# ForeverFancy/GVFDiffusion

Hardware: AMD Instinct MI355X
Metric: 4D frames/sec (800x800x24f, 256k Gaussians) + DiT denoise steps/sec (higher is better)
Workload: dtype f32

## Files before the change

gvfdiffusion_amd/csrc/rast.hip:

```cpp
#include <atomic>
#include <cstdlib>
#include <mutex>
#include <type_traits>
#include <vector>
#include "gvf_common.h"
#include "gvf_sort.h"
#include "../../include/gvf_rast.h"

namespace {

constexpr int PRE_THREADS = 256;
constexpr int NSLAB = 1;
#ifndef GVF_PRE_FB
#define GVF_PRE_FB 4
#endif
constexpr int PRE_FB = GVF_PRE_FB;
#ifndef GVF_PRE_XCD
#define GVF_PRE_XCD 0
#endif
#ifndef GVF_PRE_REC_QUAD
#define GVF_PRE_REC_QUAD 1
#endif
#ifndef GVF_PRE_PREFETCH
#define GVF_PRE_PREFETCH 0
// ... 31 lines not shown
    const float s1 = __builtin_fmaf(-l11, px, __builtin_fmaf(-l12, py, c1));
    const float s2 = __builtin_fmaf(-l22, py, c2);
    return __builtin_fmaf(s2, s2, __builtin_fmaf(s1, s1, -lo));
}

__constant__ float SH_C0 = 0.28209479177387814f;
__constant__ float SH_C1 = 0.4886025119029199f;
__constant__ float SH_C2[5] = {1.0925484305920792f, -1.0925484305920792f, 0.31539156525252005f,
                               -1.0925484305920792f, 0.5462742152960396f};
__constant__ float SH_C3[7] = {-0.5900435899266435f, 2.890611442640554f, -0.4570457994644658f,
                               0.3731763325901154f, -0.4570457994644658f, 1.445305721320277f,
                               -0.5900435899266435f};

struct PreParams {
    int P, M, deg, H, W, mode;
    int gx, gy;
    float kernel_size, scale_modifier;
    int fused;
    GvfGaussianActivation act;
    int n_delta;
    int upstream_binning;
    int F;
    int delta_lds;
};

__device__ __forceinline__ float act_expf(float x) {
    if (x != x) return x;
    if (x > 88.72283f) return __builtin_inff();
    if (x < -103.97208f) return 0.0f;
    const float kf = x * 1.44269502f + (x < 0.0f ? -0.5f : 0.5f);
    const int k = (int)kf;
    const float t = (float)k;
    float r = __builtin_fmaf(t, -0.693145751953125f, x);
    r = __builtin_fmaf(t, -1.42860677e-6f, r);
    float p = 1.98412698e-4f;
    p = __builtin_fmaf(p, r, 1.38888889e-3f);
    p = __builtin_fmaf(p, r, 8.33333377e-3f);
    p = __builtin_fmaf(p, r, 4.16666679e-2f);
    p = __builtin_fmaf(p, r, 1.66666672e-1f);
    p = __builtin_fmaf(p, r, 0.5f);
    p = __builtin_fmaf(p, r, 1.0f);
    p = __builtin_fmaf(p, r, 1.0f);
    const int k1 = k / 2, k2 = k - k1;
    return (p * __uint_as_float((uint32_t)(k1 + 127) << 23)) * __uint_as_float((uint32_t)(k2 + 127) << 23);
}
__device__ __forceinline__ float act_log1pf(float y) {
// ... 226 lines not shown
__device__ __forceinline__ void tight_range(float c, float h, int lo, int hi, int n, int& t0, int& t1) {
    if (h < 0.0f) { t0 = lo; t1 = lo; return; }
    const float a = fminf(fmaxf(ceilf((c - h - (float)(TILE - 1)) / (float)TILE), 0.0f), (float)n);
    const float b = fminf(fmaxf(floorf((c + h) / (float)TILE) + 1.0f, 0.0f), (float)n);
    t0 = max((int)a, lo);
    t1 = min((int)b, hi);
    if (t1 < t0) t1 = t0;
}

__device__ __forceinline__ TileRect tight_rect(TileRect r, float px, float py, float hx, float hy, int gx, int gy) {
    TileRect t;
    tight_range(px, hx, r.x0, r.x1, gx, t.x0, t.x1);
    tight_range(py, hy, r.y0, r.y1, gy, t.y0, t.y1);
    return t;
}

template <bool SHARED>
__global__ __launch_bounds__(PRE_THREADS) void preprocess_kernel(
    PreParams pp, const GvfRastFrame* __restrict__ frames, const float* __restrict__ a0,
    const float* __restrict__ a1, const float* __restrict__ a2, const float* __restrict__ a3,
    const float* __restrict__ sh, const float* __restrict__ colors_precomp,
    const float* __restrict__ cov3D_precomp, const float* __restrict__ delta, float4* __restrict__ splats,
    uint32_t* __restrict__ tiles_touched,
    int32_t* __restrict__ radii, uint32_t* __restrict__ block_sums, uint4* __restrict__ binrec,
    const uint32_t* __restrict__ bin_slot ,
    const float2* __restrict__ zrange ) {
    extern __shared__ __attribute__((aligned(16))) float sh_lds[];
    const int t = threadIdx.x;
    const int P = pp.P, M = pp.M;
    const int nbx = (P + PRE_THREADS - 1) / PRE_THREADS;
    int bx = blockIdx.x, by = blockIdx.y;
    if (GVF_PRE_XCD) {
        const int FY = (pp.F + PRE_FB - 1) / PRE_FB, k = (int)(blockIdx.x >> 3);
        bx = (k / FY) * 8 + (int)(blockIdx.x & 7u);
        by = k - (k / FY) * FY;
        if (bx >= nbx) return;
    }
    const int i = bx * PRE_THREADS + t;

    const int sh_stride = M * 3;
    if (sh != nullptr) {
        const size_t span0 = (size_t)bx * PRE_THREADS * sh_stride;
        const int nvalid = min(PRE_THREADS, P - bx * PRE_THREADS);
        const int total = nvalid * sh_stride;
        const float4* src4 = reinterpret_cast<const float4*>(sh + span0);
        float4* dst4 = reinterpret_cast<float4*>(sh_lds);
        const int n4 = total >> 2;
// ... 224 lines not shown
        const size_t o = (size_t)f * P + i;
#if defined(PRE_ABL_NOREC)
        if (touched != 0 && gA.x == 12345.678f) splats[4 * o] = gA;
#else
        if (!GVF_PRE_REC_QUAD && touched != 0) {
            float4* rec = splats + 4 * o;
            rec[0] = gA; rec[1] = gB; rec[2] = gC;
        }
#endif
        if (tiles_touched != nullptr) tiles_touched[o] = touched;
        if (radii != nullptr) {
            const uint32_t* gid_of = SHARED ? reinterpret_cast<const uint32_t*>(a1) : nullptr;
            radii[gid_of != nullptr ? (size_t)f * P + gid_of[i] : o] = radius_out;
        }
        if (binrec != nullptr) {
            uint32_t slab = 0u;
            if (zrange != nullptr) {
                const float2 zr = zrange[f];
                slab = (uint32_t)fminf(fmaxf((gC.y - zr.x) * zr.y, 0.0f), (float)(NSLAB - 1));
            }
#if defined(PRE_ABL_NOBIN)
            if (gC.y == 12345.678f)
#endif
            binrec[(size_t)f * P + my_slot] = make_uint4((uint32_t)rect.x0 | ((uint32_t)rect.y0 << 16),
                                                         (uint32_t)rect.x1 | ((uint32_t)rect.y1 << 16), __float_as_uint(gC.y), slab);
        }
    }

#if !defined(PRE_ABL_NOREC)
    if (GVF_PRE_REC_QUAD) {
        const int lj = t & 3;
        float4* qbase = splats + 4 * ((size_t)f * P + (size_t)(i & ~3));
#define GVF_QB(v_, k_) __builtin_bit_cast(float, __builtin_amdgcn_mov_dpp(__builtin_bit_cast(int, (v_)), (k_) * 0x55, 0xF, 0xF, true))
#define GVF_QSTORE(k_)                                                                                          \
        {                                                                                                       \
            const int tk = __builtin_amdgcn_mov_dpp((int)touched, (k_) * 0x55, 0xF, 0xF, true);                 \
            float4 o4;                                                                                          \
            { const float a = GVF_QB(gA.x, k_), b = GVF_QB(gB.x, k_), c = GVF_QB(gC.x, k_); o4.x = lj == 0 ? a : (lj == 1 ? b : (lj == 2 ? c : 0.f)); } \
            { const float a = GVF_QB(gA.y, k_), b = GVF_QB(gB.y, k_), c = GVF_QB(gC.y, k_); o4.y = lj == 0 ? a : (lj == 1 ? b : (lj == 2 ? c : 0.f)); } \
            { const float a = GVF_QB(gA.z, k_), b = GVF_QB(gB.z, k_), c = GVF_QB(gC.z, k_); o4.z = lj == 0 ? a : (lj == 1 ? b : (lj == 2 ? c : 0.f)); } \
            { const float a = GVF_QB(gA.w, k_), b = GVF_QB(gB.w, k_), c = GVF_QB(gC.w, k_); o4.w = lj == 0 ? a : (lj == 1 ? b : (lj == 2 ? c : 0.f)); } \
            if (tk != 0) qbase[4 * (k_) + lj] = o4;                                                             \
        }
        GVF_QSTORE(0) GVF_QSTORE(1) GVF_QSTORE(2) GVF_QSTORE(3)
#undef GVF_QSTORE
#undef GVF_QB
    }
#endif
// ... 180 lines not shown
    float lo[3], hi[3];
#pragma unroll
    for (int k = 0; k < 3; ++k) {
        lo[k] = float_unordered(mm[k]); hi[k] = float_unordered(mm[3 + k]);
        if (fused) { lo[k] = lo[k] * act.aabb[3 + k] + act.aabb[k]; hi[k] = hi[k] * act.aabb[3 + k] + act.aabb[k]; }
        if (lo[k] > hi[k]) { const float tmp = lo[k]; lo[k] = hi[k]; hi[k] = tmp; }
    }
    const float* V = frames[f].viewmatrix;
    float zmin = 3.0e38f, zmax = -3.0e38f;
    for (int c = 0; c < 8; ++c) {
        const float p[3] = {(c & 1) ? hi[0] : lo[0], (c & 2) ? hi[1] : lo[1], (c & 4) ? hi[2] : lo[2]};
        const float z = V[2] * p[0] + V[6] * p[1] + V[10] * p[2] + V[14];
        zmin = fminf(zmin, z); zmax = fmaxf(zmax, z);
    }
    zmin = fmaxf(zmin, 0.2f);
    const float ext = fmaxf(zmax - zmin, 1e-6f);
    zrange[f] = make_float2(zmin - 0.02f * ext, (float)NSLAB / (1.04f * ext));
}

constexpr int WIN_MAX = 2048;
constexpr int BIN_SPT = 4;
constexpr int BIN_SLOTS = PRE_THREADS * BIN_SPT;

template <bool SCATTER>
__global__ __launch_bounds__(PRE_THREADS) void bin_kernel(int P, int gx, int gy, const uint4* __restrict__ binrec,
                                                          const uint32_t* __restrict__ order,
                                                          uint32_t* __restrict__ tile_count ,
                                                          uint32_t* __restrict__ cursor ,
                                                          const uint32_t* __restrict__ total,
                                                          uint64_t* __restrict__ payload, int nslab,
                                                          const uint32_t* __restrict__ frame_base, uint32_t* __restrict__ num_rendered,
                                                          int rec_by_id, int xcd_frames, int F) {
    __shared__ uint32_t s_tab[WIN_MAX];
    __shared__ uint32_t s_run[SCATTER ? WIN_MAX : 1];
    __shared__ int s_box[4];
    int blk = (int)blockIdx.x, f = (int)blockIdx.y;
    if (xcd_frames) {
        const int nblk = (P + BIN_SLOTS - 1) / BIN_SLOTS, k = (int)(blockIdx.x >> 3);
        f = (k / nblk) * 8 + (int)(blockIdx.x & 7u);
        blk = k - (k / nblk) * nblk;
        if (f >= F) return;
    }
    if (SCATTER && num_rendered != nullptr && blk == 0 && threadIdx.x == 0)
        num_rendered[f] = frame_base[f + 1] - frame_base[f];
    if (SCATTER && *total == 0u) return;
    const int t = threadIdx.x, lane = t & 63;
    if (t == 0) { s_box[0] = 0x7fffffff; s_box[1] = 0x7fffffff; s_box[2] = 0; s_box[3] = 0; }
    int x0[BIN_SPT], y0[BIN_SPT], x1[BIN_SPT], y1[BIN_SPT], sl[BIN_SPT];
    uint64_t key[BIN_SPT];
    int bx0 = 0x7fffffff, by0 = 0x7fffffff, bx1 = 0, by1 = 0;
#pragma unroll
    for (int k = 0; k < BIN_SPT; ++k) {
        const int s = blk * BIN_SLOTS + k * PRE_THREADS + t;
        x0[k] = y0[k] = x1[k] = y1[k] = 0; sl[k] = 0; key[k] = 0;
        if (s < P) {
            const uint32_t id = order != nullptr ? order[s] : (uint32_t)s;
            const uint4 br = binrec[(size_t)f * P + (rec_by_id ? id : (uint32_t)s)];
            x0[k] = (int)(br.x & 0xffffu); y0[k] = (int)(br.x >> 16);
            x1[k] = (int)(br.y & 0xffffu); y1[k] = (int)(br.y >> 16);
            sl[k] = (int)br.w;
            key[k] = ((uint64_t)br.z << 32) | id;
            if (x1[k] > x0[k] && y1[k] > y0[k]) {
                bx0 = min(bx0, x0[k]); by0 = min(by0, y0[k]); bx1 = max(bx1, x1[k]); by1 = max(by1, y1[k]);
            } else {
                x1[k] = x0[k];
            }
        }
    }
#pragma unroll
    for (int d = 32; d >= 1; d >>= 1) {
        bx0 = min(bx0, __shfl_xor(bx0, d, 64)); by0 = min(by0, __shfl_xor(by0, d, 64));
        bx1 = max(bx1, __shfl_xor(bx1, d, 64)); by1 = max(by1, __shfl_xor(by1, d, 64));
    }
    __syncthreads();
    if (lane == 0 && bx1 > bx0) {
        atomicMin(&s_box[0], bx0); atomicMin(&s_box[1], by0); atomicMax(&s_box[2], bx1); atomicMax(&s_box[3], by1);
    }
    __syncthreads();
    const int wx0 = s_box[0], wy0 = s_box[1], ww = s_box[2] - s_box[0], wh = s_box[3] - s_box[1];
    if (ww <= 0 || wh <= 0) return;
// ... 23 lines not shown
                for (int y = y0[k]; y < y1[k]; ++y)
                    for (int x = x0[k]; x < x1[k]; ++x) {
                        const int e = ((y - wy0) * ww + (x - wx0)) * nslab + sl[k];
                        payload[s_tab[e] + atomicAdd(&s_run[e], 1u)] = key[k];
                    }
        }
    } else {
#pragma unroll
        for (int k = 0; k < BIN_SPT; ++k)
            for (int y = y0[k]; y < y1[k]; ++y)
                for (int x = x0[k]; x < x1[k]; ++x) {
                    const uint32_t pos = atomicAdd(&gtab[(y * gx + x) * nslab + sl[k]], 1u);
                    if (SCATTER) payload[pos] = key[k];
                }
    }
}

constexpr int BINX_THREADS = 512;
constexpr int BINX_TAB = 4096;
constexpr int BINX_PER_WG = 8192;
constexpr int BINX_SPT = 4;

template <bool SCATTER>
__global__ __launch_bounds__(BINX_THREADS) void bin_index_kernel(int P, int gx, const uint4* __restrict__ binrec,
                                                                 uint32_t* __restrict__ tile_count ,
                                                                 uint32_t* __restrict__ cursor ,
                                                                 const uint32_t* __restrict__ total,
                                                                 uint64_t* __restrict__ payload, int nslab, int nseg_frame,
                                                                 const uint32_t* __restrict__ frame_base, uint32_t* __restrict__ num_rendered) {
    __shared__ uint32_t s_tab[BINX_TAB];
    __shared__ uint32_t s_run[SCATTER ? BINX_TAB : 1];
    const int t = threadIdx.x, f = blockIdx.y;
    if (SCATTER && num_rendered != nullptr && blockIdx.x == 0 && t == 0) num_rendered[f] = frame_base[f + 1] - frame_base[f];
    if (SCATTER && *total == 0u) return;
    const int g0 = (int)blockIdx.x * BINX_PER_WG, g1 = min(P, g0 + BINX_PER_WG);
    const uint4* rec = binrec + (size_t)f * P;
    for (int e = t; e < nseg_frame; e += BINX_THREADS) { s_tab[e] = 0u; if (SCATTER) s_run[e] = 0u; }
    __syncthreads();
    auto sweep = [&](auto pass) {
        for (int base = g0; base < g1; base += BINX_SPT * BINX_THREADS) {
            uint4 br[BINX_SPT];
#pragma unroll
            for (int k = 0; k < BINX_SPT; ++k) {
                const int s = base + k * BINX_THREADS + t;
                br[k] = s < g1 ? rec[s] : make_uint4(0u, 0u, 0u, 0u);
            }
#pragma unroll
            for (int k = 0; k < BINX_SPT; ++k) {
                const int x0 = (int)(br[k].x & 0xffffu), y0 = (int)(br[k].x >> 16);
                const int x1 = (int)(br[k].y & 0xffffu), y1 = (int)(br[k].y >> 16);
                const int sl = (int)br[k].w;
                const uint64_t key = ((uint64_t)br[k].z << 32) | (uint32_t)(base + k * BINX_THREADS + t);
                for (int y = y0; y < y1; ++y)
                    for (int x = x0; x < x1; ++x) {
                        const int e = (y * gx + x) * nslab + sl;
                        if constexpr (decltype(pass)::value == 0) atomicAdd(&s_tab[e], 1u);
                        else payload[s_tab[e] + atomicAdd(&s_run[e], 1u)] = key;
                    }
            }
        }
    };
    sweep(std::integral_constant<int, 0>{});
    __syncthreads();
    uint32_t* gtab = (SCATTER ? cursor : tile_count) + (size_t)f * nseg_frame;
    for (int e = t; e < nseg_frame; e += BINX_THREADS) {
        const uint32_t c = s_tab[e];
        if (c != 0u) {
            if (SCATTER) s_tab[e] = atomicAdd(&gtab[e], c);
            else atomicAdd(&gtab[e], c);
        }
    }
    if (SCATTER) {
        __syncthreads();
        sweep(std::integral_constant<int, 1>{});
    }
}

__global__ __launch_bounds__(256) void bbox_kernel(int P, const float* __restrict__ xyz, uint32_t* __restrict__ mm) {
    __shared__ uint32_t s_mm[6];
    if (threadIdx.x < 6) s_mm[threadIdx.x] = threadIdx.x < 3 ? 0xffffffffu : 0u;
    __syncthreads();
    uint32_t lo[3] = {0xffffffffu, 0xffffffffu, 0xffffffffu}, hi[3] = {0u, 0u, 0u};
    for (int i = blockIdx.x * blockDim.x + threadIdx.x; i < P; i += gridDim.x * blockDim.x) {
#pragma unroll
        for (int k = 0; k < 3; ++k) {
            const float v = xyz[3 * (size_t)i + k];
            if (v == v && fabsf(v) < 3.0e38f) {
                const uint32_t o = float_ordered(v);
                lo[k] = min(lo[k], o); hi[k] = max(hi[k], o);
            }
        }
    }
#pragma unroll
    for (int k = 0; k < 3; ++k) {
#pragma unroll
        for (int d = 32; d >= 1; d >>= 1) {
            lo[k] = min(lo[k], (uint32_t)__shfl_xor((int)lo[k], d, 64));
            hi[k] = max(hi[k], (uint32_t)__shfl_xor((int)hi[k], d, 64));
        }
        if ((threadIdx.x & 63) == 0) { atomicMin(&s_mm[k], lo[k]); atomicMax(&s_mm[3 + k], hi[k]); }
    }
    __syncthreads();
    if (threadIdx.x < 3) atomicMin(&mm[threadIdx.x], s_mm[threadIdx.x]);
    else if (threadIdx.x < 6) atomicMax(&mm[threadIdx.x], s_mm[threadIdx.x]);
}

__device__ __forceinline__ uint32_t spread5(uint32_t v) {
    return (v & 1u) | ((v & 2u) << 2) | ((v & 4u) << 4) | ((v & 8u) << 6) | ((v & 16u) << 8);
}

constexpr int MORTON_BINS = 1 << 15;

__device__ __forceinline__ uint32_t morton15(int i, const float* __restrict__ xyz, const uint32_t* __restrict__ mm) {
    uint32_t code = 0;
#pragma unroll
    for (int k = 0; k < 3; ++k) {
        const float lo = float_unordered(mm[k]), hi = float_unordered(mm[3 + k]);
        const float v = xyz[3 * (size_t)i + k];
        float q = (v - lo) / fmaxf(hi - lo, 1e-30f) * 32.0f;
        q = (q == q) ? fminf(fmaxf(q, 0.0f), 31.0f) : 0.0f;
        code |= spread5((uint32_t)q) << k;
    }
    return code;
}

__global__ __launch_bounds__(256) void morton_count_kernel(int P, const float* __restrict__ xyz,
                                                           const uint32_t* __restrict__ mm, uint32_t* __restrict__ codes,
                                                           uint32_t* __restrict__ hist) {
    const int i = blockIdx.x * blockDim.x + threadIdx.x;
    if (i >= P) return;
    const uint32_t c = morton15(i, xyz, mm);
    codes[i] = c;
    atomicAdd(&hist[c], 1u);
}

__global__ __launch_bounds__(1024) void morton_scan_kernel(uint32_t* __restrict__ hist) {
    __shared__ uint32_t wsum[16];
    const int t = threadIdx.x;
    const unsigned lane = t & 63, w = t >> 6;
    constexpr int PER = MORTON_BINS / 1024;
    uint32_t v[PER], s = 0;
#pragma unroll
    for (int k = 0; k < PER; ++k) { v[k] = hist[t * PER + k]; s += v[k]; }
    const uint32_t incl = gvf_wave_incl_scan(s, lane);
    if (lane == 63) wsum[w] = incl;
    __syncthreads();
    uint32_t run = incl - s;
    for (unsigned k = 0; k < w; ++k) run += wsum[k];
#pragma unroll
    for (int k = 0; k < PER; ++k) { hist[t * PER + k] = run; run += v[k]; }
}

__global__ __launch_bounds__(256) void morton_scatter_kernel(int P, uint32_t* codes_rank, uint32_t* __restrict__ hist,
                                                             uint32_t* __restrict__ order) {
    const int i = blockIdx.x * blockDim.x + threadIdx.x;
    if (i >= P) return;
    const uint32_t slot = atomicAdd(&hist[codes_rank[i]], 1u);
    order[slot] = (uint32_t)i;
    codes_rank[i] = slot;
}

__global__ __launch_bounds__(256) void ranges_kernel(const uint64_t* __restrict__ keys,
                                                     const uint32_t* __restrict__ n_ptr, uint32_t n_cap,
                                                     uint2* __restrict__ ranges, uint32_t n_ranges) {
    uint32_t n = *n_ptr;
    n = n < n_cap ? n : n_cap;
    for (uint32_t k = blockIdx.x * blockDim.x + threadIdx.x; k < n; k += gridDim.x * blockDim.x) {
        uint32_t cur = (uint32_t)(keys[k] >> 32);
        if (cur >= n_ranges) continue;
        if (k == 0) ranges[cur].x = 0;
        else {
            uint32_t prev = (uint32_t)(keys[k - 1] >> 32);
            if (cur != prev) { if (prev < n_ranges) ranges[prev].y = k; ranges[cur].x = k; }
        }
        if (k == n - 1) ranges[cur].y = n;
    }
}

#ifndef SORT_BUCKETS
#define SORT_BUCKETS 1
#endif

// ... 680 lines not shown

constexpr int PROF_MAX_CALLS = 256;
constexpr int PROF_EVENTS = GVF_RAST_NSTAGES + 1;
struct Profiler {
    bool on = false;
    std::atomic<int> calls{0};
    hipEvent_t ev[PROF_MAX_CALLS][PROF_EVENTS];
};
Profiler g_prof;
inline void prof_mark(hipStream_t s, int slot, int k) {
    if (slot >= 0) (void)hipEventRecord(g_prof.ev[slot][k], s);
}

struct Workspace {
    GvfRastFrame* frames;
    float4* splats;
    uint32_t* tiles_touched; int32_t* radii;
    uint32_t* block_sums; uint32_t* frame_base; uint32_t* total;
    uint64_t* keys; uint64_t* keys_alt; uint32_t* vals; uint32_t* vals_alt; uint32_t* ids;
    uint2* ranges; uint32_t* cls;
    uint32_t* tile_count; uint32_t* cursor;
    uint32_t* partial; float2* zrange;
    uint32_t* order; uint32_t* order_alt; uint32_t* mhist; uint32_t* mm;
    uint4* binrec;
    void* sort_tmp; size_t sort_tmp_bytes;
    size_t bytes; bool ok;
};

int key_end_bit(int F, int ntiles) {
    uint64_t m = (uint64_t)F * (uint64_t)ntiles;
    int bits = 0;
    while (((uint64_t)1 << bits) < m) ++bits;
    return 32 + bits;
}

Workspace carve(void* ws, size_t bytes, int P, int F, int H, int W, int64_t max_rendered) {
    Workspace w;
    GvfCarver c(ws, bytes);
    const int nb = (P + PRE_THREADS - 1) / PRE_THREADS;
    const int ntiles = ((W + TILE - 1) / TILE) * ((H + TILE - 1) / TILE);
    const size_t FP = (size_t)F * (size_t)(P > 0 ? P : 1);
    const size_t D = (size_t)(max_rendered > 0 ? max_rendered : 1);
    w.frames = c.take<GvfRastFrame>(F);
    w.splats = c.take<float4>(4 * FP);
    w.tiles_touched = c.take<uint32_t>(FP);
    w.radii = c.take<int32_t>(FP);
    w.block_sums = c.take<uint32_t>((size_t)F * (nb > 0 ? nb : 1));
    w.frame_base = c.take<uint32_t>(F + 1);
    w.total = c.take<uint32_t>(1);
    w.keys = c.take<uint64_t>(D);
    w.keys_alt = c.take<uint64_t>(D);
    w.vals = c.take<uint32_t>(D);
    w.vals_alt = c.take<uint32_t>(D);
    w.ids = c.take<uint32_t>(D);
    w.ranges = c.take<uint2>((size_t)F * ntiles * NSLAB);
    w.cls = c.take<uint32_t>(2 + 2 * (size_t)F * ntiles * NSLAB);
    w.tile_count = c.take<uint32_t>((size_t)F * ntiles * NSLAB);
    w.cursor = c.take<uint32_t>((size_t)F * ntiles * NSLAB);
    w.partial = c.take<uint32_t>(((size_t)F * ntiles * NSLAB + SCAN_CHUNK - 1) / SCAN_CHUNK + 1);
    w.zrange = c.take<float2>(F);
    const size_t Pp = (size_t)(P > 0 ? P : 1);
    w.order = c.take<uint32_t>(Pp);
    w.order_alt = c.take<uint32_t>(Pp);
    w.mhist = c.take<uint32_t>(1 << 15);
    w.mm = c.take<uint32_t>(8);
    w.binrec = c.take<uint4>(FP);
    w.sort_tmp_bytes = gvf_sort_tmp_bytes((int64_t)D);
    w.sort_tmp = c.take<char>(w.sort_tmp_bytes);
    w.bytes = gvf_align_up(c.off, 256);
    w.ok = c.ok;
    return w;
}

std::atomic<long long> g_shared_calls{0};

int run_pipeline(const GvfRastSettings& st, const GvfRastFrame* frames_host, int F, int P, int M, bool fused,
                 const GvfGaussianActivation* act, const float* a0, const float* a1, const float* a2,
                 const float* a3, const float* sh, const float* colors_precomp, const float* cov3D_precomp,
                 const float* delta, int n_delta, const float* subpixel_offset, void* workspace,
                 size_t workspace_bytes, int64_t max_rendered, float* out_color, float* out_alpha,
                 float* out_depth, int32_t* out_radii, uint32_t* out_num_rendered, hipStream_t stream,
                 unsigned char* out_u8 = nullptr ) {
    const int H = st.image_height, W = st.image_width;
    if (H <= 0 || W <= 0 || P < 0 || F <= 0 || max_rendered < 0 || max_rendered > 0xFFFFFFFFll) return GVF_EINVAL;
    if (st.sh_degree < 0 || st.sh_degree > 3) return GVF_EINVAL;
    if (st.mode != GVF_RAST_MODE_MIP && st.mode != GVF_RAST_MODE_DILATE) return GVF_EINVAL;
    if ((out_color == nullptr) == (out_u8 == nullptr) || !out_num_rendered || !frames_host || !workspace) return GVF_EINVAL;
    if (P > 0 && colors_precomp == nullptr) {
        if (sh == nullptr || M < (st.sh_degree + 1) * (st.sh_degree + 1) || M > MAX_SH_COEFFS) return GVF_EINVAL;
    }
    (void)hipGetLastError();
    if ((((uintptr_t)sh) & 15) != 0 || (((uintptr_t)workspace) & 255) != 0) return GVF_EINVAL;
    Workspace w = carve(workspace, workspace_bytes, P, F, H, W, max_rendered);
    if (!w.ok) return GVF_ENOSPC;

    const int gx = (W + TILE - 1) / TILE, gy = (H + TILE - 1) / TILE, ntiles = gx * gy;
    const int nb = (P + PRE_THREADS - 1) / PRE_THREADS;
    int slot = g_prof.on ? g_prof.calls.fetch_add(1) : -1;
    if (slot >= PROF_MAX_CALLS) slot = -1;

    ActSlices slices; slices.n = 0;
    bool shared = false;
    std::vector<int> frame_slice((size_t)F, 0);
    const char* shared_env = getenv("GVF_RAST_SHARED_ACT");
    const bool shared_on = !(shared_env && shared_env[0] == '0');
    if (shared_on && fused && cov3D_precomp == nullptr && st.bin_algo != GVF_RAST_BIN_RADIX && P > 0 && F >= 2) {
        shared = true;
        for (int f = 0; f < F && shared; ++f) {
            const int di = (delta != nullptr && frames_host[f].delta_index >= 0) ? frames_host[f].delta_index : -1;
            int k = 0;
            while (k < slices.n && slices.di[k] != di) ++k;
            if (k == slices.n) {
                if (slices.n == ACT_MAX_SLICES) { shared = false; break; }
                slices.di[slices.n++] = di;
            }
            frame_slice[(size_t)f] = k;
        }
        if (shared && (F < 2 * slices.n || (size_t)slices.n * (size_t)P * 64u > (size_t)(max_rendered > 0 ? max_rendered : 0) * 8u)) shared = false;
    }
    const bool index_fits = st.bin_algo != GVF_RAST_BIN_RADIX && !shared && (size_t)ntiles * NSLAB <= (size_t)BINX_TAB;
    const bool index_count = GVF_BIN_ALGO >= 2 && index_fits, index_scatter = GVF_BIN_ALGO == 3 && index_fits;
    const bool morton = st.bin_algo != GVF_RAST_BIN_RADIX && F >= 4 && P >= 4096 && !index_scatter;
    const char* slot_env = getenv("GVF_RAST_SLOT_ORDER");
    const size_t sh_floats = (size_t)(colors_precomp ? 0 : M) * 3;
    const bool slot_mode = shared && !(slot_env && slot_env[0] == '0') && morton && nb > 0 && colors_precomp == nullptr && sh != nullptr &&
                           (size_t)slices.n * (size_t)P * 64u + (size_t)P * sh_floats * 4u <= (size_t)max_rendered * 8u;
    const uint32_t layout = (slot_mode ? LAYOUT_SLOT_ORDER : 0u) | ((uint32_t)((P > 0 && nb > 0 && morton) ? NSLAB : 1) << 8);
    for (int f0 = 0; f0 < F; f0 += 16) {
        FrameChunk ch;
        const int cnt = F - f0 < 16 ? F - f0 : 16;
        for (int k = 0; k < cnt; ++k) {
            ch.f[k] = frames_host[f0 + k];
            ch.f[k].reserved[0] = shared ? frame_slice[(size_t)(f0 + k)] : 0;
        }
        CallTables tab = {};
        if (f0 == 0) {
            const size_t nseg_all = (size_t)F * ntiles * NSLAB;
            tab.ranges = reinterpret_cast<uint32_t*>(w.ranges); tab.n_ranges = (uint32_t)(2 * nseg_all);
            tab.tile_count = w.tile_count; tab.n_tile_count = (uint32_t)nseg_all;
            tab.mhist = w.mhist; tab.n_mhist = morton ? (uint32_t)MORTON_BINS : 0u;
            tab.cls = w.cls; tab.mm = w.mm; tab.layout = layout;
        }
        const size_t clear_words = (size_t)tab.n_ranges + tab.n_tile_count + tab.n_mhist;
        const int zb = f0 == 0 ? (int)((clear_words + 4095) / 4096 < 256 ? (clear_words + 4095) / 4096 : 256) : 0;
        hipLaunchKernelGGL(upload_frames_kernel, dim3(1 + zb), dim3(256), 0, stream, ch, cnt, w.frames + f0, tab);
    }
    GVF_CHECK_LAUNCH();

    int nslab_blend = 1;
    const uint32_t* blend_rec_of = nullptr;
    if (P == 0 || nb == 0) {
        if (hipMemsetAsync(out_num_rendered, 0, sizeof(uint32_t) * F, stream) != hipSuccess) return GVF_ELAUNCH;
    } else {
        const bool bucket = st.bin_algo != GVF_RAST_BIN_RADIX;
        prof_mark(stream, slot, 0);
        const uint32_t* order = nullptr;
        if (morton) {
            int bb = (P + 255) / 256; if (bb > 128) bb = 128;
            const int pb = (P + 255) / 256;
            hipLaunchKernelGGL(bbox_kernel, dim3(bb), dim3(256), 0, stream, P, a0, w.mm);
            hipLaunchKernelGGL(morton_count_kernel, dim3(pb), dim3(256), 0, stream, P, a0, w.mm, w.order_alt, w.mhist);
            hipLaunchKernelGGL(morton_scan_kernel, dim3(1), dim3(1024), 0, stream, w.mhist);
            hipLaunchKernelGGL(morton_scatter_kernel, dim3(pb), dim3(256), 0, stream, P, w.order_alt, w.mhist, w.order);
            order = w.order;
            if (NSLAB > 1)
                hipLaunchKernelGGL(frame_zrange_kernel, dim3((F + 63) / 64), dim3(64), 0, stream, w.frames, F, w.mm, fused ? 1 : 0,
                                   fused ? *act : GvfGaussianActivation{}, w.zrange);
            GVF_CHECK_LAUNCH();
        }
        const int nslab = order != nullptr ? NSLAB : 1;
        const bool rec_gather = GVF_BIN_ALGO >= 1 && bucket && !shared && order != nullptr;
        nslab_blend = nslab;
        const unsigned nseg = (unsigned)((size_t)F * ntiles * nslab);
        prof_mark(stream, slot, 1);
        PreParams pp;
        pp.P = P; pp.M = colors_precomp ? 0 : M; pp.deg = st.sh_degree; pp.H = H; pp.W = W; pp.mode = st.mode;
        pp.gx = gx; pp.gy = gy; pp.kernel_size = st.kernel_size; pp.scale_modifier = st.scale_modifier;
        pp.fused = fused ? 1 : 0; pp.n_delta = n_delta; pp.F = F;
        pp.upstream_binning = (st.upstream_binning != 0 || subpixel_offset != nullptr) ? 1 : 0;
        if (fused) pp.act = *act; else pp.act = GvfGaussianActivation{};
        const size_t sh_lds_bytes = gvf_align_up((size_t)PRE_THREADS * pp.M * 3 * sizeof(float), 16) + 16;
        pp.delta_lds = (GVF_PRE_DELTA_LDS && fused && delta != nullptr && P % 2 == 0 && (((uintptr_t)delta) & 15) == 0) ? 1 : 0;
        const size_t pre_lds_bytes = sh_lds_bytes + (pp.delta_lds ? (size_t)PRE_THREADS * 14 * sizeof(float) : 0);
        const int pre_fy = (F + PRE_FB - 1) / PRE_FB;
        const dim3 pre_grid = GVF_PRE_XCD ? dim3((nb + 7) / 8 * 8 * pre_fy) : dim3(nb, pre_fy);
        if (shared) {
            g_shared_calls.fetch_add(1, std::memory_order_relaxed);
            float4* rec3d = reinterpret_cast<float4*>(w.keys_alt);
            float* sh_by_slot = slot_mode ? reinterpret_cast<float*>(rec3d + 4 * (size_t)slices.n * (size_t)P) : nullptr;
            hipLaunchKernelGGL(activate_cov_kernel, dim3((P + 255) / 256, slices.n), dim3(256), 0, stream, *act, st.scale_modifier, P, slices,
                               a0, a1, a2, a3, delta, rec3d, slot_mode ? w.order_alt : nullptr, sh, (int)sh_floats, sh_by_slot);
            if (slot_mode) {
                blend_rec_of = w.order_alt;
                hipLaunchKernelGGL(preprocess_kernel<true>, pre_grid, dim3(PRE_THREADS), sh_lds_bytes, stream, pp,
                                   w.frames, reinterpret_cast<const float*>(rec3d), reinterpret_cast<const float*>(order), nullptr, nullptr, sh_by_slot,
                                   nullptr, nullptr, nullptr, w.splats, nullptr, out_radii == nullptr ? nullptr : w.radii, nullptr, w.binrec,
                                   nullptr, nslab > 1 ? w.zrange : nullptr);
            } else
            hipLaunchKernelGGL(preprocess_kernel<true>, pre_grid, dim3(PRE_THREADS), sh_lds_bytes, stream, pp,
                               w.frames, reinterpret_cast<const float*>(rec3d), nullptr, nullptr, nullptr, colors_precomp ? nullptr : sh, colors_precomp,
                               nullptr, nullptr, w.splats, nullptr, out_radii == nullptr ? nullptr : w.radii, nullptr, w.binrec,
                               order != nullptr ? w.order_alt : nullptr, nslab > 1 ? w.zrange : nullptr);
        } else
        hipLaunchKernelGGL(preprocess_kernel<false>, pre_grid, dim3(PRE_THREADS), pre_lds_bytes, stream, pp,
                           w.frames, a0, a1, a2, a3, colors_precomp ? nullptr : sh, colors_precomp, cov3D_precomp, delta,
                           w.splats, bucket ? nullptr : w.tiles_touched, (bucket && out_radii == nullptr) ? nullptr : w.radii,
                           bucket ? nullptr : w.block_sums, bucket ? w.binrec : nullptr,
                           (order != nullptr && !rec_gather) ? w.order_alt : nullptr, (bucket && nslab > 1) ? w.zrange : nullptr);
        const int bnb = (P + BIN_SLOTS - 1) / BIN_SLOTS, xnb = (P + BINX_PER_WG - 1) / BINX_PER_WG;
        const dim3 bin_grid = rec_gather ? dim3((unsigned)((F + 7) / 8 * 8 * bnb)) : dim3(bnb, F);
        if (index_count)
            hipLaunchKernelGGL(bin_index_kernel<false>, dim3(xnb, F), dim3(BINX_THREADS), 0, stream, P, gx, w.binrec,
                               w.tile_count, w.cursor, w.total, w.keys, nslab, ntiles * nslab, nullptr, nullptr);
        else if (bucket)
            hipLaunchKernelGGL(bin_kernel<false>, bin_grid, dim3(PRE_THREADS), 0, stream, P, gx, gy, w.binrec, order,
                               w.tile_count, w.cursor, w.total, w.keys, nslab, nullptr, nullptr, rec_gather ? 1 : 0, rec_gather ? 1 : 0, F);
        GVF_CHECK_LAUNCH();
        prof_mark(stream, slot, 2);
        if (bucket)
        {
            const int sblocks = (int)((nseg + SCAN_CHUNK - 1) / SCAN_CHUNK);
            hipLaunchKernelGGL(seg_sums_kernel, dim3(sblocks), dim3(1024), 0, stream, w.tile_count, (int)nseg, w.partial);
            hipLaunchKernelGGL(seg_scan_kernel, dim3(sblocks), dim3(1024), 0, stream, w.tile_count, (int)nseg, ntiles * nslab, F,
                               w.partial, sblocks, w.ranges, w.cursor, w.frame_base, out_num_rendered, w.total,
                               (uint32_t)max_rendered, w.cls);
            if (max_rendered <= 0)
                hipLaunchKernelGGL(frame_counts_kernel, dim3((F + 63) / 64), dim3(64), 0, stream, w.frame_base, F, out_num_rendered);
        }
        else
            hipLaunchKernelGGL(scan_sums_kernel, dim3(1), dim3(1024), 0, stream, w.block_sums, nb, F, w.frame_base,
                               out_num_rendered, w.total, (uint32_t)max_rendered);
        GVF_CHECK_LAUNCH();
        prof_mark(stream, slot, 3);
        if (max_rendered > 0) {
            if (index_scatter)
                hipLaunchKernelGGL(bin_index_kernel<true>, dim3(xnb, F), dim3(BINX_THREADS), 0, stream, P, gx, w.binrec,
                                   w.tile_count, w.cursor, w.total, w.keys, nslab, ntiles * nslab, w.frame_base, out_num_rendered);
            else if (bucket)
                hipLaunchKernelGGL(bin_kernel<true>, bin_grid, dim3(PRE_THREADS), 0, stream, P, gx, gy, w.binrec, order,
                                   w.tile_count, w.cursor, w.total, w.keys, nslab, w.frame_base, out_num_rendered,
                                   rec_gather ? 1 : 0, rec_gather ? 1 : 0, F);
            else
                hipLaunchKernelGGL(duplicate_kernel, dim3(nb, F), dim3(PRE_THREADS), 0, stream, P, gx, gy, w.splats,
                                   w.tiles_touched, w.radii, w.block_sums, w.keys, w.vals, (uint32_t)max_rendered,
                                   pp.upstream_binning);
            GVF_CHECK_LAUNCH();
        }
        if (out_radii != nullptr) {
            if (hipMemcpyAsync(out_radii, w.radii, sizeof(int32_t) * (size_t)F * P, hipMemcpyDeviceToDevice, stream) != hipSuccess)
                return GVF_ELAUNCH;
        }
        prof_mark(stream, slot, 4);
        if (max_rendered > 0) {
            uint64_t* keys_sorted = w.keys;
            uint32_t* vals_by_tile = nullptr;
            if (!bucket) {
                vals_by_tile = w.vals;
                int in_alt = 0;
                int rc = gvf_sort_pairs_device_n(w.keys, w.keys_alt, w.vals, w.vals_alt, w.total, max_rendered, 32,
                                                 key_end_bit(F, ntiles), w.sort_tmp, w.sort_tmp_bytes, stream, &in_alt);
                if (rc != GVF_OK) return rc;
                if (in_alt) { keys_sorted = w.keys_alt; vals_by_tile = w.vals_alt; }
// ... 942 lines not shown
```

Measured before the change: 20840.

## Compress bin records to 8 bytes and rebuild Morton ordering with LDS histograms

Bin records now pack tile rectangles into 8-bit fields (8 bytes per record instead of 16) whenever the tile grid fits in 255x255 and only one depth slab is used, which halves the traffic written by preprocess and read by the binning kernels. The Morton reorder path is also rebuilt: bbox reduction uses float4 loads and writes per-block partials instead of global atomics, the code drops to 12 bits, and the histogram and ranking run as two 1024-thread kernels using LDS histograms and LDS rank assignment instead of global per-element atomics. Together these cut bandwidth and atomic contention in the preprocessing front end, at the cost of a coarser spatial ordering and a different order within each bin.

```diff
diff --git a/gvfdiffusion_amd/csrc/rast.hip b/gvfdiffusion_amd/csrc/rast.hip
--- a/gvfdiffusion_amd/csrc/rast.hip
+++ b/gvfdiffusion_amd/csrc/rast.hip
@@ -77,6 +77,7 @@
     int upstream_binning;
     int F;
     int delta_lds;
+    int rec8;
 };
 
 __device__ __forceinline__ float act_expf(float x) {
@@ -349,7 +350,7 @@
     const float* __restrict__ sh, const float* __restrict__ colors_precomp,
     const float* __restrict__ cov3D_precomp, const float* __restrict__ delta, float4* __restrict__ splats,
     uint32_t* __restrict__ tiles_touched,
-    int32_t* __restrict__ radii, uint32_t* __restrict__ block_sums, uint4* __restrict__ binrec,
+    int32_t* __restrict__ radii, uint32_t* __restrict__ block_sums, void* __restrict__ binrec ,
     const uint32_t* __restrict__ bin_slot ,
     const float2* __restrict__ zrange ) {
     extern __shared__ __attribute__((aligned(16))) float sh_lds[];
@@ -620,8 +621,15 @@
 #if defined(PRE_ABL_NOBIN)
             if (gC.y == 12345.678f)
 #endif
-            binrec[(size_t)f * P + my_slot] = make_uint4((uint32_t)rect.x0 | ((uint32_t)rect.y0 << 16),
-                                                         (uint32_t)rect.x1 | ((uint32_t)rect.y1 << 16), __float_as_uint(gC.y), slab);
+            {
+            const size_t ro = (size_t)f * P + my_slot;
+            if (pp.rec8)
+                static_cast<uint2*>(binrec)[ro] = make_uint2((uint32_t)rect.x0 | ((uint32_t)rect.y0 << 8) | ((uint32_t)rect.x1 << 16) |
+                                                                 ((uint32_t)rect.y1 << 24), __float_as_uint(gC.y));
+            else
+                static_cast<uint4*>(binrec)[ro] = make_uint4((uint32_t)rect.x0 | ((uint32_t)rect.y0 << 16),
+                                                             (uint32_t)rect.x1 | ((uint32_t)rect.y1 << 16), __float_as_uint(gC.y), slab);
+            }
         }
     }
 
@@ -848,8 +856,16 @@
 constexpr int BIN_SPT = 4;
 constexpr int BIN_SLOTS = PRE_THREADS * BIN_SPT;
 
+__device__ __forceinline__ uint4 binrec_load(const void* __restrict__ binrec, int rec8, size_t k) {
+    if (rec8) {
+        const uint2 r = static_cast<const uint2*>(binrec)[k];
+        return make_uint4((r.x & 0xffu) | ((r.x & 0xff00u) << 8), ((r.x >> 16) & 0xffu) | ((r.x >> 8) & 0xff0000u), r.y, 0u);
+    }
+    return static_cast<const uint4*>(binrec)[k];
+}
+
 template <bool SCATTER>
-__global__ __launch_bounds__(PRE_THREADS) void bin_kernel(int P, int gx, int gy, const uint4* __restrict__ binrec,
+__global__ __launch_bounds__(PRE_THREADS) void bin_kernel(int P, int gx, int gy, const void* __restrict__ binrec, int rec8,
                                                           const uint32_t* __restrict__ order,
                                                           uint32_t* __restrict__ tile_count ,
                                                           uint32_t* __restrict__ cursor ,
@@ -881,7 +897,7 @@
         x0[k] = y0[k] = x1[k] = y1[k] = 0; sl[k] = 0; key[k] = 0;
         if (s < P) {
             const uint32_t id = order != nullptr ? order[s] : (uint32_t)s;
-            const uint4 br = binrec[(size_t)f * P + (rec_by_id ? id : (uint32_t)s)];
+            const uint4 br = binrec_load(binrec, rec8, (size_t)f * P + (rec_by_id ? id : (uint32_t)s));
             x0[k] = (int)(br.x & 0xffffu); y0[k] = (int)(br.x >> 16);
             x1[k] = (int)(br.y & 0xffffu); y1[k] = (int)(br.y >> 16);
             sl[k] = (int)br.w;
@@ -951,7 +967,7 @@
 constexpr int BINX_SPT = 4;
 
 template <bool SCATTER>
-__global__ __launch_bounds__(BINX_THREADS) void bin_index_kernel(int P, int gx, const uint4* __restrict__ binrec,
+__global__ __launch_bounds__(BINX_THREADS) void bin_index_kernel(int P, int gx, const void* __restrict__ binrec, int rec8,
                                                                  uint32_t* __restrict__ tile_count ,
                                                                  uint32_t* __restrict__ cursor ,
                                                                  const uint32_t* __restrict__ total,
@@ -963,7 +979,7 @@
     if (SCATTER && num_rendered != nullptr && blockIdx.x == 0 && t == 0) num_rendered[f] = frame_base[f + 1] - frame_base[f];
     if (SCATTER && *total == 0u) return;
     const int g0 = (int)blockIdx.x * BINX_PER_WG, g1 = min(P, g0 + BINX_PER_WG);
-    const uint4* rec = binrec + (size_t)f * P;
+    const size_t rec0 = (size_t)f * P;
     for (int e = t; e < nseg_frame; e += BINX_THREADS) { s_tab[e] = 0u; if (SCATTER) s_run[e] = 0u; }
     __syncthreads();
     auto sweep = [&](auto pass) {
@@ -972,7 +988,7 @@
 #pragma unroll
             for (int k = 0; k < BINX_SPT; ++k) {
                 const int s = base + k * BINX_THREADS + t;
-                br[k] = s < g1 ? rec[s] : make_uint4(0u, 0u, 0u, 0u);
+                br[k] = s < g1 ? binrec_load(binrec, rec8, rec0 + s) : make_uint4(0u, 0u, 0u, 0u);
             }
 #pragma unroll
             for (int k = 0; k < BINX_SPT; ++k) {
@@ -1005,20 +1021,34 @@
     }
 }
 
-__global__ __launch_bounds__(256) void bbox_kernel(int P, const float* __restrict__ xyz, uint32_t* __restrict__ mm) {
+constexpr int BBOX_BLOCKS = 256;
+__global__ __launch_bounds__(256) void bbox_kernel(int P, const float* __restrict__ xyz, uint32_t* __restrict__ part) {
     __shared__ uint32_t s_mm[6];
     if (threadIdx.x < 6) s_mm[threadIdx.x] = threadIdx.x < 3 ? 0xffffffffu : 0u;
     __syncthreads();
     uint32_t lo[3] = {0xffffffffu, 0xffffffffu, 0xffffffffu}, hi[3] = {0u, 0u, 0u};
-    for (int i = blockIdx.x * blockDim.x + threadIdx.x; i < P; i += gridDim.x * blockDim.x) {
-#pragma unroll
-        for (int k = 0; k < 3; ++k) {
-            const float v = xyz[3 * (size_t)i + k];
-            if (v == v && fabsf(v) < 3.0e38f) {
-                const uint32_t o = float_ordered(v);
-                lo[k] = min(lo[k], o); hi[k] = max(hi[k], o);
-            }
-        }
+    auto acc = [&](int k, float v) {
+        if (v == v && fabsf(v) < 3.0e38f) {
+            const uint32_t o = float_ordered(v);
+            lo[k] = min(lo[k], o); hi[k] = max(hi[k], o);
+        }
+    };
+    const int t0 = blockIdx.x * blockDim.x + threadIdx.x, stride = gridDim.x * blockDim.x;
+    int tail0 = 0;
+    if ((((uintptr_t)xyz) & 15) == 0) {
+        const float4* x4 = reinterpret_cast<const float4*>(xyz);
+        const int nq = P >> 2;
+        for (int q = t0; q < nq; q += stride) {
+            const float4 a = x4[3 * (size_t)q], b = x4[3 * (size_t)q + 1], c = x4[3 * (size_t)q + 2];
+            acc(0, a.x); acc(1, a.y); acc(2, a.z); acc(0, a.w);
+            acc(1, b.x); acc(2, b.y); acc(0, b.z); acc(1, b.w);
+            acc(2, c.x); acc(0, c.y); acc(1, c.z); acc(2, c.w);
+        }
+        tail0 = nq << 2;
+    }
+    for (int i = tail0 + t0; i < P; i += stride) {
+#pragma unroll
+        for (int k = 0; k < 3; ++k) acc(k, xyz[3 * (size_t)i + k]);
     }
 #pragma unroll
     for (int k = 0; k < 3; ++k) {
@@ -1030,63 +1060,163 @@
         if ((threadIdx.x & 63) == 0) { atomicMin(&s_mm[k], lo[k]); atomicMax(&s_mm[3 + k], hi[k]); }
     }
     __syncthreads();
-    if (threadIdx.x < 3) atomicMin(&mm[threadIdx.x], s_mm[threadIdx.x]);
-    else if (threadIdx.x < 6) atomicMax(&mm[threadIdx.x], s_mm[threadIdx.x]);
-}
-
-__device__ __forceinline__ uint32_t spread5(uint32_t v) {
-    return (v & 1u) | ((v & 2u) << 2) | ((v & 4u) << 4) | ((v & 8u) << 6) | ((v & 16u) << 8);
-}
-
-constexpr int MORTON_BINS = 1 << 15;
-
-__device__ __forceinline__ uint32_t morton15(int i, const float* __restrict__ xyz, const uint32_t* __restrict__ mm) {
+    if (threadIdx.x < 6) part[threadIdx.x * BBOX_BLOCKS + blockIdx.x] = s_mm[threadIdx.x];
+}
+
+#ifndef GVF_MORTON_BITS
+#define GVF_MORTON_BITS 4
+#endif
+__device__ __forceinline__ uint32_t spread_bits(uint32_t v) {
+    uint32_t r = 0;
+#pragma unroll
+    for (int b = 0; b < GVF_MORTON_BITS; ++b) r |= ((v >> b) & 1u) << (3 * b);
+    return r;
+}
+
+constexpr int MORTON_CELLS = 1 << GVF_MORTON_BITS;
+constexpr bool MORTON_LDS_RANK = GVF_MORTON_BITS == 4;
+constexpr int MORTON_BINS = MORTON_CELLS * MORTON_CELLS * MORTON_CELLS;
+constexpr int MORTON_THREADS = 1024;
+#ifndef GVF_MORTON_PT
+#define GVF_MORTON_PT 8
+#endif
+constexpr int MORTON_PT = GVF_MORTON_PT;
+constexpr int MORTON_PER_WG = MORTON_THREADS * MORTON_PT;
+constexpr int MORTON_PER = MORTON_BINS / MORTON_THREADS;
+static_assert(MORTON_PER % 4 == 0, "morton_rank_kernel scans whole uint4 of bins");
+
+__device__ __forceinline__ uint32_t morton12(int i, const float* __restrict__ xyz, const float (&lo)[3], const float (&ext)[3]) {
     uint32_t code = 0;
 #pragma unroll
     for (int k = 0; k < 3; ++k) {
-        const float lo = float_unordered(mm[k]), hi = float_unordered(mm[3 + k]);
         const float v = xyz[3 * (size_t)i + k];
-        float q = (v - lo) / fmaxf(hi - lo, 1e-30f) * 32.0f;
-        q = (q == q) ? fminf(fmaxf(q, 0.0f), 31.0f) : 0.0f;
-        code |= spread5((uint32_t)q) << k;
+        float q = (v - lo[k]) / ext[k] * (float)MORTON_CELLS;
+        q = (q == q) ? fminf(fmaxf(q, 0.0f), (float)(MORTON_CELLS - 1)) : 0.0f;
+        code |= spread_bits((uint32_t)q) << k;
     }
     return code;
 }
 
-__global__ __launch_bounds__(256) void morton_count_kernel(int P, const float* __restrict__ xyz,
-                                                           const uint32_t* __restrict__ mm, uint32_t* __restrict__ codes,
-                                                           uint32_t* __restrict__ hist) {
-    const int i = blockIdx.x * blockDim.x + threadIdx.x;
-    if (i >= P) return;
-    const uint32_t c = morton15(i, xyz, mm);
-    codes[i] = c;
-    atomicAdd(&hist[c], 1u);
-}
-
-__global__ __launch_bounds__(1024) void morton_scan_kernel(uint32_t* __restrict__ hist) {
-    __shared__ uint32_t wsum[16];
+__global__ __launch_bounds__(MORTON_THREADS) void morton_hist_kernel(int P, const float* __restrict__ xyz, const uint32_t* __restrict__ part,
+                                                                     int nbb, uint32_t* __restrict__ mm, uint32_t* __restrict__ codes,
+                                                                     uint32_t* __restrict__ hist) {
+    __shared__ uint32_t s_h[MORTON_BINS];
+    __shared__ uint32_t s_mm[6];
+    const int t = threadIdx.x;
+    for (int b = t; b < MORTON_BINS; b += MORTON_THREADS) s_h[b] = 0u;
+    if (t < 6) s_mm[t] = t < 3 ? 0xffffffffu : 0u;
+    __syncthreads();
+    if (t < BBOX_BLOCKS) {
+        uint32_t v[6];
+#pragma unroll
+        for (int k = 0; k < 6; ++k) v[k] = t < nbb ? part[k * BBOX_BLOCKS + t] : (k < 3 ? 0xffffffffu : 0u);
+#pragma unroll
+        for (int d = 32; d >= 1; d >>= 1) {
+#pragma unroll
+            for (int k = 0; k < 3; ++k) {
+                v[k] = min(v[k], (uint32_t)__shfl_xor((int)v[k], d, 64));
+                v[3 + k] = max(v[3 + k], (uint32_t)__shfl_xor((int)v[3 + k], d, 64));
+            }
+        }
+        if ((t & 63) == 0) {
+#pragma unroll
+            for (int k = 0; k < 3; ++k) { atomicMin(&s_mm[k], v[k]); atomicMax(&s_mm[3 + k], v[3 + k]); }
+        }
+    }
+    __syncthreads();
+    if (blockIdx.x == 0 && t < 6) mm[t] = s_mm[t];
+    float lo[3], ext[3];
+#pragma unroll
+    for (int k = 0; k < 3; ++k) {
+        lo[k] = float_unordered(s_mm[k]);
+        ext[k] = fmaxf(float_unordered(s_mm[3 + k]) - lo[k], 1e-30f);
+    }
+    const int g0 = (int)blockIdx.x * MORTON_PER_WG;
+#pragma unroll
+    for (int k = 0; k < MORTON_PT; ++k) {
+        const int i = g0 + k * MORTON_THREADS + t;
+        if (i < P) {
+            const uint32_t c = morton12(i, xyz, lo, ext);
+            codes[i] = c;
+            atomicAdd(&s_h[c], 1u);
+        }
+    }
+    __syncthreads();
+    for (int b = t; b < MORTON_BINS; b += MORTON_THREADS) {
+        const uint32_t c = s_h[b];
+        if (c != 0u) atomicAdd(&hist[b], c);
+    }
+}
+
+__global__ __launch_bounds__(MORTON_THREADS) void morton_rank_kernel(int P, const uint32_t* __restrict__ hist, uint32_t* __restrict__ cursor,
+                                                                     uint32_t* __restrict__ codes_rank, uint32_t* __restrict__ order) {
+    __shared__ uint32_t s_base[MORTON_BINS];
+    __shared__ uint32_t s_cnt[MORTON_LDS_RANK ? MORTON_BINS : 1];
+    __shared__ uint32_t s_wsum[MORTON_THREADS / GVF_WAVE];
     const int t = threadIdx.x;
     const unsigned lane = t & 63, w = t >> 6;
-    constexpr int PER = MORTON_BINS / 1024;
-    uint32_t v[PER], s = 0;
-#pragma unroll
-    for (int k = 0; k < PER; ++k) { v[k] = hist[t * PER + k]; s += v[k]; }
+    uint4 v[MORTON_PER / 4];
+    uint32_t s = 0;
+#pragma unroll
+    for (int j = 0; j < MORTON_PER / 4; ++j) {
+        v[j] = reinterpret_cast<const uint4*>(hist)[t * (MORTON_PER / 4) + j];
+        s += v[j].x + v[j].y + v[j].z + v[j].w;
+    }
     const uint32_t incl = gvf_wave_incl_scan(s, lane);
-    if (lane == 63) wsum[w] = incl;
+    if (lane == 63) s_wsum[w] = incl;
+    if (MORTON_LDS_RANK)
+        for (int b = t; b < MORTON_BINS; b += MORTON_THREADS) s_cnt[b] = 0u;
     __syncthreads();
     uint32_t run = incl - s;
-    for (unsigned k = 0; k < w; ++k) run += wsum[k];
-#pragma unroll
-    for (int k = 0; k < PER; ++k) { hist[t * PER + k] = run; run += v[k]; }
-}
-
-__global__ __launch_bounds__(256) void morton_scatter_kernel(int P, uint32_t* codes_rank, uint32_t* __restrict__ hist,
-                                                             uint32_t* __restrict__ order) {
-    const int i = blockIdx.x * blockDim.x + threadIdx.x;
-    if (i >= P) return;
-    const uint32_t slot = atomicAdd(&hist[codes_rank[i]], 1u);
-    order[slot] = (uint32_t)i;
-    codes_rank[i] = slot;
+    for (unsigned k = 0; k < w; ++k) run += s_wsum[k];
+#pragma unroll
+    for (int j = 0; j < MORTON_PER / 4; ++j) {
+        uint32_t* sb = s_base + t * MORTON_PER + 4 * j;
+        sb[0] = run; run += v[j].x;
+        sb[1] = run; run += v[j].y;
+        sb[2] = run; run += v[j].z;
+        sb[3] = run; run += v[j].w;
+    }
+    const int g0 = (int)blockIdx.x * MORTON_PER_WG;
+    if (!MORTON_LDS_RANK) {
+        __syncthreads();
+#pragma unroll
+        for (int k = 0; k < MORTON_PT; ++k) {
+            const int i = g0 + k * MORTON_THREADS + t;
+            if (i < P) {
+                const uint32_t c = codes_rank[i] & (MORTON_BINS - 1);
+                const uint32_t slot = s_base[c] + atomicAdd(&cursor[c], 1u);
+                if (slot < (uint32_t)P) order[slot] = (uint32_t)i;
+                codes_rank[i] = slot;
+            }
+        }
+        return;
+    }
+    uint32_t code[MORTON_PT], rank[MORTON_PT];
+#pragma unroll
+    for (int k = 0; k < MORTON_PT; ++k) {
+        const int i = g0 + k * MORTON_THREADS + t;
+        code[k] = 0u; rank[k] = 0u;
+        if (i < P) {
+            code[k] = codes_rank[i] & (MORTON_BINS - 1);
+            rank[k] = atomicAdd(&s_cnt[code[k]], 1u);
+        }
+    }
+    __syncthreads();
+    for (int b = t; b < MORTON_BINS; b += MORTON_THREADS) {
+        const uint32_t c = s_cnt[b];
+        if (c != 0u) s_base[b] += atomicAdd(&cursor[b], c);
+    }
+    __syncthreads();
+#pragma unroll
+    for (int k = 0; k < MORTON_PT; ++k) {
+        const int i = g0 + k * MORTON_THREADS + t;
+        if (i < P) {
+            const uint32_t slot = s_base[code[k]] + rank[k];
+            if (slot < (uint32_t)P) order[slot] = (uint32_t)i;
+            codes_rank[i] = slot;
+        }
+    }
 }
 
 __global__ __launch_bounds__(256) void ranges_kernel(const uint64_t* __restrict__ keys,
@@ -1813,7 +1943,7 @@
     uint32_t* tile_count; uint32_t* cursor;
     uint32_t* partial; float2* zrange;
     uint32_t* order; uint32_t* order_alt; uint32_t* mhist; uint32_t* mm;
-    uint4* binrec;
+    void* binrec;
     void* sort_tmp; size_t sort_tmp_bytes;
     size_t bytes; bool ok;
 };
@@ -1825,7 +1955,7 @@
     return 32 + bits;
 }
 
-Workspace carve(void* ws, size_t bytes, int P, int F, int H, int W, int64_t max_rendered) {
+Workspace carve(void* ws, size_t bytes, int P, int F, int H, int W, int64_t max_rendered, int rec_bytes = 16) {
     Workspace w;
     GvfCarver c(ws, bytes);
     const int nb = (P + PRE_THREADS - 1) / PRE_THREADS;
@@ -1853,11 +1983,11 @@
     const size_t Pp = (size_t)(P > 0 ? P : 1);
     w.order = c.take<uint32_t>(Pp);
     w.order_alt = c.take<uint32_t>(Pp);
-    w.mhist = c.take<uint32_t>(1 << 15);
+    w.mhist = c.take<uint32_t>(2 * MORTON_BINS + 6 * BBOX_BLOCKS);
     w.mm = c.take<uint32_t>(8);
-    w.binrec = c.take<uint4>(FP);
     w.sort_tmp_bytes = gvf_sort_tmp_bytes((int64_t)D);
     w.sort_tmp = c.take<char>(w.sort_tmp_bytes);
+    w.binrec = c.take<char>(FP * (size_t)rec_bytes);
     w.bytes = gvf_align_up(c.off, 256);
     w.ok = c.ok;
     return w;
@@ -1882,10 +2012,12 @@
     }
     (void)hipGetLastError();
     if ((((uintptr_t)sh) & 15) != 0 || (((uintptr_t)workspace) & 255) != 0) return GVF_EINVAL;
-    Workspace w = carve(workspace, workspace_bytes, P, F, H, W, max_rendered);
+    const int gx = (W + TILE - 1) / TILE, gy = (H + TILE - 1) / TILE, ntiles = gx * gy;
+    const char* rec16_env = getenv("GVF_RAST_BINREC16");
+    const bool rec8 = NSLAB == 1 && gx <= 255 && gy <= 255 && !(rec16_env && rec16_env[0] == '1');
+    Workspace w = carve(workspace, workspace_bytes, P, F, H, W, max_rendered, rec8 ? 8 : 16);
     if (!w.ok) return GVF_ENOSPC;
 
-    const int gx = (W + TILE - 1) / TILE, gy = (H + TILE - 1) / TILE, ntiles = gx * gy;
     const int nb = (P + PRE_THREADS - 1) / PRE_THREADS;
     int slot = g_prof.on ? g_prof.calls.fetch_add(1) : -1;
     if (slot >= PROF_MAX_CALLS) slot = -1;
@@ -1929,7 +2061,7 @@
             const size_t nseg_all = (size_t)F * ntiles * NSLAB;
             tab.ranges = reinterpret_cast<uint32_t*>(w.ranges); tab.n_ranges = (uint32_t)(2 * nseg_all);
             tab.tile_count = w.tile_count; tab.n_tile_count = (uint32_t)nseg_all;
-            tab.mhist = w.mhist; tab.n_mhist = morton ? (uint32_t)MORTON_BINS : 0u;
+            tab.mhist = w.mhist; tab.n_mhist = morton ? (uint32_t)(2 * MORTON_BINS) : 0u;
             tab.cls = w.cls; tab.mm = w.mm; tab.layout = layout;
         }
         const size_t clear_words = (size_t)tab.n_ranges + tab.n_tile_count + tab.n_mhist;
@@ -1947,12 +2079,15 @@
         prof_mark(stream, slot, 0);
         const uint32_t* order = nullptr;
         if (morton) {
-            int bb = (P + 255) / 256; if (bb > 128) bb = 128;
-            const int pb = (P + 255) / 256;
-            hipLaunchKernelGGL(bbox_kernel, dim3(bb), dim3(256), 0, stream, P, a0, w.mm);
-            hipLaunchKernelGGL(morton_count_kernel, dim3(pb), dim3(256), 0, stream, P, a0, w.mm, w.order_alt, w.mhist);
-            hipLaunchKernelGGL(morton_scan_kernel, dim3(1), dim3(1024), 0, stream, w.mhist);
-            hipLaunchKernelGGL(morton_scatter_kernel, dim3(pb), dim3(256), 0, stream, P, w.order_alt, w.mhist, w.order);
+            int bb = (P / 4 + 255) / 256;
+            bb = bb < 1 ? 1 : (bb > BBOX_BLOCKS ? BBOX_BLOCKS : bb);
+            const int mb = (P + MORTON_PER_WG - 1) / MORTON_PER_WG;
+            uint32_t* bbox_part = w.mhist + 2 * MORTON_BINS;
+            hipLaunchKernelGGL(bbox_kernel, dim3(bb), dim3(256), 0, stream, P, a0, bbox_part);
+            hipLaunchKernelGGL(morton_hist_kernel, dim3(mb), dim3(MORTON_THREADS), 0, stream, P, a0, bbox_part, bb, w.mm, w.order_alt,
+                               w.mhist);
+            hipLaunchKernelGGL(morton_rank_kernel, dim3(mb), dim3(MORTON_THREADS), 0, stream, P, w.mhist, w.mhist + MORTON_BINS,
+                               w.order_alt, w.order);
             order = w.order;
             if (NSLAB > 1)
                 hipLaunchKernelGGL(frame_zrange_kernel, dim3((F + 63) / 64), dim3(64), 0, stream, w.frames, F, w.mm, fused ? 1 : 0,
@@ -1967,7 +2102,7 @@
         PreParams pp;
         pp.P = P; pp.M = colors_precomp ? 0 : M; pp.deg = st.sh_degree; pp.H = H; pp.W = W; pp.mode = st.mode;
         pp.gx = gx; pp.gy = gy; pp.kernel_size = st.kernel_size; pp.scale_modifier = st.scale_modifier;
-        pp.fused = fused ? 1 : 0; pp.n_delta = n_delta; pp.F = F;
+        pp.fused = fused ? 1 : 0; pp.n_delta = n_delta; pp.F = F; pp.rec8 = rec8 ? 1 : 0;
         pp.upstream_binning = (st.upstream_binning != 0 || subpixel_offset != nullptr) ? 1 : 0;
         if (fused) pp.act = *act; else pp.act = GvfGaussianActivation{};
         const size_t sh_lds_bytes = gvf_align_up((size_t)PRE_THREADS * pp.M * 3 * sizeof(float), 16) + 16;
@@ -2001,10 +2136,10 @@
         const int bnb = (P + BIN_SLOTS - 1) / BIN_SLOTS, xnb = (P + BINX_PER_WG - 1) / BINX_PER_WG;
         const dim3 bin_grid = rec_gather ? dim3((unsigned)((F + 7) / 8 * 8 * bnb)) : dim3(bnb, F);
         if (index_count)
-            hipLaunchKernelGGL(bin_index_kernel<false>, dim3(xnb, F), dim3(BINX_THREADS), 0, stream, P, gx, w.binrec,
+            hipLaunchKernelGGL(bin_index_kernel<false>, dim3(xnb, F), dim3(BINX_THREADS), 0, stream, P, gx, w.binrec, pp.rec8,
                                w.tile_count, w.cursor, w.total, w.keys, nslab, ntiles * nslab, nullptr, nullptr);
         else if (bucket)
-            hipLaunchKernelGGL(bin_kernel<false>, bin_grid, dim3(PRE_THREADS), 0, stream, P, gx, gy, w.binrec, order,
+            hipLaunchKernelGGL(bin_kernel<false>, bin_grid, dim3(PRE_THREADS), 0, stream, P, gx, gy, w.binrec, pp.rec8, order,
                                w.tile_count, w.cursor, w.total, w.keys, nslab, nullptr, nullptr, rec_gather ? 1 : 0, rec_gather ? 1 : 0, F);
         GVF_CHECK_LAUNCH();
         prof_mark(stream, slot, 2);
@@ -2025,10 +2160,10 @@
         prof_mark(stream, slot, 3);
         if (max_rendered > 0) {
             if (index_scatter)
-                hipLaunchKernelGGL(bin_index_kernel<true>, dim3(xnb, F), dim3(BINX_THREADS), 0, stream, P, gx, w.binrec,
+                hipLaunchKernelGGL(bin_index_kernel<true>, dim3(xnb, F), dim3(BINX_THREADS), 0, stream, P, gx, w.binrec, pp.rec8,
                                    w.tile_count, w.cursor, w.total, w.keys, nslab, ntiles * nslab, w.frame_base, out_num_rendered);
             else if (bucket)
-                hipLaunchKernelGGL(bin_kernel<true>, bin_grid, dim3(PRE_THREADS), 0, stream, P, gx, gy, w.binrec, order,
+                hipLaunchKernelGGL(bin_kernel<true>, bin_grid, dim3(PRE_THREADS), 0, stream, P, gx, gy, w.binrec, pp.rec8, order,
                                    w.tile_count, w.cursor, w.total, w.keys, nslab, w.frame_base, out_num_rendered,
                                    rec_gather ? 1 : 0, rec_gather ? 1 : 0, F);
             else
```

Result: faster. 21110, median of 6 (+1.3%).
